# Xjh-UCAS/TAM-TR

Measured on AMD Instinct MI355X. Metric: images/sec fwd+bwd @640x640 bs=16/GPU, higher is better.
Workload: dtype bf16

## Files before the change

### include/tamtr_hip.h

```cpp
#ifndef TAMTR_HIP_H
#define TAMTR_HIP_H

#include <stdint.h>

#ifdef __cplusplus
extern "C" {
#endif

#define TAMTR_F32 0
#define TAMTR_BF16 1

#define TAMTR_OK 0
#define TAMTR_EINVAL (-1)
#define TAMTR_EUNSUP (-2)
#define TAMTR_ELAUNCH (-3)

int tamtr_abi_version(void);

int tamtr_maxsigmoid_gate_fwd(const void* x, const float* gk, const float* bias, const void* v, void* out, float* aw,
                              int32_t* arg, int B, int nh, int hc, int HW, int T, float scale, int dtype, void* stream);

int tamtr_maxsigmoid_gate_bwd(const void* dout, const void* x, const float* gk, const void* v, const float* aw,
                              const int32_t* arg, void* dx, void* dv, float* dlogit, int B, int nh, int hc, int HW, int T,
                              float scale, int dtype, void* stream);
int tamtr_maxsigmoid_gate_cl_fwd(const void* e, long long ld_e, const float* mean_rstd_e, const float* gamma_e, const float* beta_e,
                                 const void* v, const float* mean_rstd_v, const float* gamma_v, const float* beta_v, const float* gk,
                                 const float* bias, void* out, float* aw, int32_t* arg, int B, int nh, int hc, int HW, int T, float scale,
                                 int dtype, void* stream);

int tamtr_conv3x3_tiles(int B, int H, int W);
int tamtr_conv3x3_pack_weight(const void* w, void* wpk, int C1, int C2, int dtype, void* stream);
int tamtr_conv3x3_cl_stats_fwd(const void* x, long long ld_x, const void* wpk, void* y, float* running_mean, float* running_var,
                               float* mean_rstd, float* partials, int B, int H, int W, int C1, int C2, float eps, float momentum,
                               void* stream);
int tamtr_bn_finalize(const float* partials, float* mean_rstd, float* running_mean, float* running_var, int C, int S, float eps,
                      float momentum, void* stream);

int tamtr_msdeform_attn_fwd(const void* value, const int32_t* shapes_host, const float* loc, const float* aw, void* out,
                            int B, int L, int M, int D, int Q, int nl, int P, int dtype, void* stream);

int tamtr_msdeform_attn_bwd(const void* gout, const void* value, const int32_t* shapes_host, const float* loc,
                            const float* aw, float* gvalue, float* gloc, float* gaw, int B, int L, int M, int D, int Q,
                            int nl, int P, int dtype, void* stream);

int tamtr_msdeform_attn_bwd_sorted(const void* gout, const void* value, const int32_t* shapes_host, const float* loc,
                                   const float* aw, void* gvalue, float* gloc, float* gaw, float* colw, int B, int L, int M,
                                   int D, int Q, int nl, int P, long long ldg, int dtype, void* stream);

int tamtr_contrastive_logits_fwd(const void* x, const float* w, const float* logit_scale, const float* bias, float* logits,
                                 float* xinv, float* winv, int B, int Q, int K, int C, int dtype, void* stream);

int tamtr_contrastive_bwd_slabs(int Q);
int tamtr_contrastive_logits_bwd(const float* g, const void* x, const float* w, const float* logit_scale, const float* xinv,
                                 const float* winv, void* dx, float* dwhat, int B, int Q, int K, int C, int dtype,
                                 void* stream);

int tamtr_linear_bf16(const void* X, const void* W, const float* bias, void* Y, int M, int N, int K, void* stream);

int tamtr_selfattn_fwd(const void* q, const void* k, const void* v, const uint32_t* mask_bits, void* o, float* lse, int B,
                       int Q, int nh, int dh, int ldq, int ldk, int ldv, int dtype, void* stream);
int tamtr_selfattn_bwd(const void* go, const void* q, const void* k, const void* v, const void* o, const float* lse,
                       const uint32_t* mask_bits, void* gq, void* gk, void* gv, float* delta_ws, int B, int Q, int nh, int dh,
                       int ldq, int ldk, int ldv, int dtype, void* stream);

int tamtr_selective_scan_chunk(void);
int tamtr_selective_scan_fwd(const float* u, const float* delta, const float* A, const float* Bm, const float* Cm,
                             const float* D, const float* dbias, float* y, float* hstate, int B, int K, int Dk, int N, int L,
                             int xmode, void* stream);
int tamtr_selective_scan_bwd_slabs(int Dk);
int tamtr_selective_scan_row_sums(void);
int tamtr_selective_scan_bwd(const float* gy, const float* u, const float* delta, const float* A, const float* Bm,
                             const float* Cm, const float* D, const float* dbias, const float* hstate, float* gu,
                             float* gdelta, float* grow, float* gB, float* gC, float* ws, int B, int K, int Dk, int N, int L,
                             int xmode, void* stream);

int tamtr_selective_scan_dtproj_fwd(const void* u, const float* dtr, const float* Wdt, const float* A, const float* Bm,
                                    const float* Cm, const float* D, const float* dbias, void* y, float* hstate, int B, int K,
                                    int Dk, int N, int R, int L, int xmode, int planes_bf16, void* stream);
int tamtr_selective_scan_dtproj_bwd(const void* gy, const void* u, const float* dtr, const float* Wdt, const float* A,
                                    const float* Bm, const float* Cm, const float* D, const float* dbias, const float* hstate,
                                    void* gu, void* gdelta_ws, float* gdtr, float* grow, float* gB, float* gC, float* ws, int B,
                                    int K, int Dk, int N, int R, int L, int xmode, int bf16_flags, void* stream);

int tamtr_lsap_assign(const float* cost, const int32_t* group_sizes_host, int bs, int nq, int G, int64_t* batch_idx,
                      int64_t* query_idx, int64_t* gt_idx, void* stream);

int tamtr_cpam_fwd(const void* x, const void* p, void* out, float* s2, int32_t* arg, int B, int C, int H, int W, int dtype,
                   void* stream);

int tamtr_cpam_bwd(const void* gout, const void* x, const void* p, const float* s2, const int32_t* arg, void* dx_direct,
                   void* du_ws, void* dp, int B, int C, int H, int W, int dtype, void* stream);

int tamtr_cpam_cl_fwd(const void* x, void* p, uint8_t* code, void* out, float* s2, int32_t* arg, int B, int C, int H, int W, int dtype, void* stream);
int tamtr_cpam_cl_bwd(const void* gout, const void* x, const void* p, const uint8_t* code, const float* s2, const int32_t* arg, void* dxd_ws,
                      void* du_ws, void* dp_ws, void* dx, int B, int C, int H, int W, int dtype, void* stream);

int tamtr_dwconv_silu_cross_fwd(const void* x, long long x_pixel_stride, const float* weight, const float* bias, void* u2, int B,
                                int D, int H, int W, int dtype, int plane_dtype, void* stream);
int tamtr_dwconv_tiles(int H, int W);
int tamtr_dwconv_silu_cross_bwd(const void* g2, const void* x, long long x_pixel_stride, const float* weight, const float* bias,
                                void* gx, long long gx_pixel_stride, float* ws, int B, int D, int H, int W, int dtype, int plane_dtype,
                                void* stream);

int tamtr_cross_merge_fwd(const void* y4, float* ymT, int B, int D, int H, int W, int plane_dtype, void* stream);
int tamtr_cross_merge_bwd(const float* gymT, void* g2, int B, int D, int H, int W, int plane_dtype, void* stream);

int tamtr_ln_gate_blocks(long long ntok);
int tamtr_ln_gate_fwd(const float* x, const void* xz, long long xz_token_stride, const float* gamma, const float* beta, void* out,
                      float* stats, long long ntok, int D, float eps, int dtype, void* stream);
int tamtr_ln_gate_bwd(const void* gout, const float* x, const void* xz, long long xz_token_stride, const float* gamma,
                      const float* beta, const float* stats, float* gx, void* gxz, float* partials, long long ntok, int D, int dtype,
                      void* stream);

int tamtr_sum_n(const void* const* src, int n, void* out, long long n_elems, int dtype, void* stream);

int tamtr_colsum_blocks(long long M);
int tamtr_colsum_bf16(const void* X, float* partial, long long M, int N, void* stream);
int tamtr_slab_sum_rows(const void* in, float* out, int R, long long C, int dtype, void* stream);
int tamtr_dw_slices(long long M, int N, int K);
int tamtr_dw_bf16(const void* dY, const void* X, float* part, int with_db, long long M, int N, int K, void* stream);
int tamtr_fold_add(const float* g4, const void* m0, const void* m1, float* out, int B, long long n, int dtype, void* stream);

int tamtr_layernorm_fwd(const void* x, const float* gamma, const float* beta, void* out, float* stats, long long ntok, int D,
                        float eps, int dtype, void* stream);
int tamtr_layernorm_bwd(const void* gout, const void* x, const float* gamma, const float* stats, void* gx, float* partials,
                        long long ntok, int D, int dtype, void* stream);

int tamtr_bn_slices(int B, int HW);
int tamtr_bn_act_fwd(const void* x, const float* gamma, const float* beta, float* running_mean, float* running_var, void* y,
                     float* mean_rstd, float* partials, int B, int C, int HW, float eps, float momentum, int act, int dtype, void* stream);
int tamtr_bn_act_bwd(const void* gy, const void* x, const float* gamma, const float* beta, const float* mean_rstd, void* gx,
                     float* ggamma, float* gbeta, float* partials, int B, int C, int HW, int act, int dtype, void* stream);

int tamtr_bncl_blocks(long long N, int C, int dtype);
int tamtr_bncl_act_fwd(const void* x, const float* gamma, const float* beta, float* running_mean, float* running_var, const void* residual,
                       void* y, float* mean_rstd, float* partials, long long N, int C, float eps, float momentum, int act, int dtype,
                       void* stream);
int tamtr_bncl_stats(const void* x, float* running_mean, float* running_var, float* mean_rstd, float* partials, long long N, int C, float eps,
                     float momentum, int dtype, void* stream);
int tamtr_bncl2_act_fwd(const void* x1, const float* gamma1, const float* beta1, float* running_mean1, float* running_var1, const void* x2,
                        const float* gamma2, const float* beta2, float* running_mean2, float* running_var2, void* y, float* mean_rstd,
                        float* partials, long long N, int C, float eps, float momentum, int act, int dtype, void* stream);
int tamtr_bncl2_act_bwd(const void* gy, long long ldgy, const void* x1, const void* x2, const float* gamma1, const float* beta1,
                        const float* gamma2, const float* beta2, const float* mean_rstd, void* gx1, void* gx2, float* ggamma1, float* gbeta1,
                        float* ggamma2, float* gbeta2, float* partials, long long N, int C, int act, int dtype, void* stream);
int tamtr_bncl_act_bwd(const void* gy, long long ldgy, const void* x, const float* gamma, const float* beta, const float* mean_rstd,
                       void* gx, float* ggamma, float* gbeta, float* partials, long long N, int C, int act, int dtype, void* stream);

int tamtr_relayout(const void* src, void* dst, int B, int C, int HW, int ld, int to_nhwc, int dtype, void* stream);
int tamtr_resample2(const void* src, void* dst, int B, int H, int W, int C, int mode, int dtype, void* stream);
int tamtr_copy_rows(const void* src, long long lds, void* dst, long long ldd, long long N, int C, int dtype, void* stream);
int tamtr_cat_rows(const void* const* src, const long long* lds, const int* C, int n, void* dst, long long ldd, long long N, int dtype,
                   void* stream);

int tamtr_maxpool_out(int n, int k, int s, int p);
int tamtr_maxpool_fwd(const void* x, void* y, uint8_t* code, int B, int C, int H, int W, int k, int s, int p, int nhwc, int dtype,
                      void* stream);
int tamtr_maxpool_bwd(const void* gy, const uint8_t* code, const void* addend, void* gx, int B, int C, int H, int W, int k, int s, int p, int nhwc, int dtype,
                      void* stream);

int tamtr_img_augment_u8(const uint8_t* src, const double* inv_affine, const uint8_t* luts, const int32_t* flags, float* out, int B,
                         int SH, int SW, int H, int W, int border, void* stream);

int tamtr_optim_chunk(void);
int tamtr_optim_step(const void* const* p, const void* const* m, const void* const* v, const void* const* e, const void* const* shadow, float* step,
                     const long long* numel,
                     const unsigned char* group, const int* chunk_tensor, const long long* chunk_off, const void* const* grads, int ntensors,
                     int nchunks, float* partial, float* normcoef, const float* lr, const float* wd, int ngroups, float beta1, float beta2, float eps,
                     float max_norm, float ema_decay, int do_ema, void* stream);

int tamtr_xproj_dw_slices(int L);
int tamtr_xproj_fwd(const void* u2, const void* wcat, float* dtr, float* Bs, float* Cs, int B, int D, int L, int R, int plane_dtype, void* stream);
int tamtr_xproj_bwd_dx(const void* gu, const float* gdtr, const float* gB, const float* gC, const void* wT, void* gu2, int B, int D, int L, int R,
                       int plane_dtype, void* stream);
int tamtr_xproj_bwd_dw(const void* u2, const float* gdtr, const float* gB, const float* gC, float* part, int B, int D, int L, int R, int plane_dtype,
                       void* stream);

int tamtr_detr_blocks(int rows_per_layer);
int tamtr_detr_layers_fwd(const float* pb, const float* ps, const float* gt_bboxes, const long long* gt_cls, const long long* li, const long long* bi,
                          const long long* si, const long long* gi, int Lr, int B, int nq, int nc, int n, long long* tgt, float* score, float* pair_l1,
                          float* pair_riou, float* partial, float g_class, float g_bbox, float g_giou, float* out, void* stream);
int tamtr_detr_layers_bwd(const float* pb, const float* ps, const float* gt_bboxes, const long long* li, const long long* bi, const long long* si,
                          const long long* gi, const long long* tgt, const float* score, const float* up, int Lr, int B, int nq, int nc, int n,
                          float g_class, float g_bbox, float g_giou, float* gpb, float* gps, void* stream);
int tamtr_detr_match_cost(const float* ps, const float* pb, const float* gt_bboxes, const long long* gt_cls, long long rows, int nc, int G, float g_class,
// ... 98 lines not shown
```

### tam-tr_amd/_lib.py

```python
import ctypes
import os
from ctypes import c_float, c_int, c_longlong, c_void_p

_HERE = os.path.dirname(os.path.abspath(__file__))
LIB_PATH = os.environ.get('TAMTR_HIP_LIB') or os.path.join(_HERE, 'csrc', 'libtamtr_hip.so')
ABI_VERSION = 36

F32, BF16 = 0, 1
_ERR = {-1: 'TAMTR_EINVAL (bad argument)', -2: 'TAMTR_EUNSUP (shape/dtype outside what the kernels are built for)',
        -3: 'TAMTR_ELAUNCH (HIP launch error)'}


class TamtrHipError(RuntimeError):
    pass


_P, _I, _F, _LL, _D = c_void_p, c_int, c_float, c_longlong, ctypes.c_double
_SIGS = {
    'tamtr_abi_version': [],
    'tamtr_maxsigmoid_gate_fwd': [_P, _P, _P, _P, _P, _P, _P, _I, _I, _I, _I, _I, _F, _I, _P],
    'tamtr_maxsigmoid_gate_bwd': [_P, _P, _P, _P, _P, _P, _P, _P, _P, _I, _I, _I, _I, _I, _F, _I, _P],
    'tamtr_msdeform_attn_fwd': [_P, _P, _P, _P, _P, _I, _I, _I, _I, _I, _I, _I, _I, _P],
    'tamtr_msdeform_attn_bwd': [_P, _P, _P, _P, _P, _P, _P, _P, _I, _I, _I, _I, _I, _I, _I, _I, _P],
    'tamtr_msdeform_attn_bwd_sorted': [_P, _P, _P, _P, _P, _P, _P, _P, _P, _I, _I, _I, _I, _I, _I, _I, _LL, _I, _P],
    'tamtr_contrastive_logits_fwd': [_P, _P, _P, _P, _P, _P, _P, _I, _I, _I, _I, _I, _P],
    'tamtr_contrastive_logits_bwd': [_P, _P, _P, _P, _P, _P, _P, _P, _I, _I, _I, _I, _I, _P],
    'tamtr_contrastive_bwd_slabs': [_I],
    'tamtr_linear_bf16': [_P, _P, _P, _P, _I, _I, _I, _P],
    'tamtr_selfattn_fwd': [_P, _P, _P, _P, _P, _P, _I, _I, _I, _I, _I, _I, _I, _I, _P],
    'tamtr_selfattn_bwd': [_P] * 11 + [_I, _I, _I, _I, _I, _I, _I, _I, _P],
    'tamtr_selective_scan_chunk': [],
    'tamtr_selective_scan_fwd': [_P, _P, _P, _P, _P, _P, _P, _P, _P, _I, _I, _I, _I, _I, _I, _P],
    'tamtr_selective_scan_bwd_slabs': [_I],
    'tamtr_selective_scan_row_sums': [],
    'tamtr_selective_scan_bwd': [_P] * 15 + [_I, _I, _I, _I, _I, _I, _P],
    'tamtr_selective_scan_dtproj_fwd': [_P] * 10 + [_I] * 8 + [_P],
    'tamtr_selective_scan_dtproj_bwd': [_P] * 17 + [_I] * 8 + [_P],
    'tamtr_lsap_assign': [_P, _P, _I, _I, _I, _P, _P, _P, _P],
    'tamtr_img_augment_u8': [_P, _P, _P, _P, _P, _I, _I, _I, _I, _I, _I, _P],
    'tamtr_cpam_fwd': [_P, _P, _P, _P, _P, _I, _I, _I, _I, _I, _P],
    'tamtr_cpam_cl_fwd': [_P, _P, _P, _P, _P, _P, _I, _I, _I, _I, _I, _P],
    'tamtr_cpam_bwd': [_P] * 8 + [_I, _I, _I, _I, _I, _P],
    'tamtr_cpam_cl_bwd': [_P] * 10 + [_I, _I, _I, _I, _I, _P],
    'tamtr_dwconv_silu_cross_fwd': [_P, _LL, _P, _P, _P, _I, _I, _I, _I, _I, _I, _P],
    'tamtr_dwconv_tiles': [_I, _I],
    'tamtr_cross_merge_fwd': [_P, _P, _I, _I, _I, _I, _I, _P],
    'tamtr_cross_merge_bwd': [_P, _P, _I, _I, _I, _I, _I, _P],
    'tamtr_ln_gate_blocks': [_LL],
    'tamtr_bn_slices': [_I, _I],
    'tamtr_maxpool_out': [_I, _I, _I, _I],
    'tamtr_maxpool_fwd': [_P, _P, _P, _I, _I, _I, _I, _I, _I, _I, _I, _I, _P],
    'tamtr_maxpool_bwd': [_P, _P, _P, _P, _I, _I, _I, _I, _I, _I, _I, _I, _I, _P],
    'tamtr_sum_n': [_P, _I, _P, _LL, _I, _P],
    'tamtr_colsum_blocks': [_LL],
    'tamtr_colsum_bf16': [_P, _P, _LL, _I, _P],
    'tamtr_fold_add': [_P, _P, _P, _P, _I, _LL, _I, _P],
    'tamtr_slab_sum_rows': [_P, _P, _I, _LL, _I, _P],
    'tamtr_dw_slices': [_LL, _I, _I],
    'tamtr_dw_bf16': [_P, _P, _P, _I, _LL, _I, _I, _P],
    'tamtr_graph_capture_census': [_P, _P, _I],
    'tamtr_box_refine_fwd': [_P, _P, _P, _LL, _P],
    'tamtr_box_refine_bwd': [_P, _P, _P, _P, _P, _LL, _P],
    'tamtr_bncl_act_seg_fwd': [_P, _P, _P, _P, _P, _P, _LL, _LL, _P, _P, _LL, _I, _F, _F, _I, _I, _P],
    'tamtr_bncl_act_seg_bwd': [_P, _LL, _LL, _P, _P, _P, _P, _P, _P, _P, _P, _LL, _I, _I, _I, _P],
    'tamtr_detr_blocks': [_I],
    'tamtr_detr_layers_fwd': [_P] * 8 + [_I] * 5 + [_P] * 5 + [_F, _F, _F, _P, _P],
    'tamtr_detr_layers_bwd': [_P] * 10 + [_I] * 5 + [_F, _F, _F, _P, _P, _P],
    'tamtr_detr_match_cost': [_P, _P, _P, _P, _LL, _I, _I, _F, _F, _F, _F, _F, _P, _P],
    'tamtr_xproj_dw_slices': [_I],
    'tamtr_xproj_fwd': [_P, _P, _P, _P, _P, _I, _I, _I, _I, _I, _P],
    'tamtr_xproj_bwd_dx': [_P, _P, _P, _P, _P, _P, _I, _I, _I, _I, _I, _P],
    'tamtr_xproj_bwd_dw': [_P, _P, _P, _P, _P, _I, _I, _I, _I, _I, _P],
    'tamtr_optim_chunk': [],
    'tamtr_optim_step': [_P] * 11 + [_I, _I, _P, _P, _P, _P, _I, _F, _F, _F, _F, _F, _I, _P],
    'tamtr_resample2': [_P, _P, _I, _I, _I, _I, _I, _I, _P],
    'tamtr_cat_rows': [_P, _P, _P, _I, _P, _LL, _LL, _I, _P],
    'tamtr_copy_rows': [_P, _LL, _P, _LL, _LL, _I, _I, _P],
    'tamtr_relayout': [_P, _P, _I, _I, _I, _I, _I, _I, _P],
    'tamtr_bncl_blocks': [_LL, _I, _I],
    'tamtr_bncl_act_fwd': [_P, _P, _P, _P, _P, _P, _P, _P, _P, _LL, _I, _F, _F, _I, _I, _P],
    'tamtr_bncl_stats': [_P, _P, _P, _P, _P, _LL, _I, _F, _F, _I, _P],
    'tamtr_bn_finalize': [_P, _P, _P, _P, _I, _I, _F, _F, _P],
    'tamtr_conv3x3_tiles': [_I, _I, _I],
    'tamtr_conv3x3_pack_weight': [_P, _P, _I, _I, _I, _P],
    'tamtr_conv3x3_cl_stats_fwd': [_P, _LL, _P, _P, _P, _P, _P, _P, _I, _I, _I, _I, _I, _F, _F, _P],
    'tamtr_maxsigmoid_gate_cl_fwd': [_P, _LL, _P, _P, _P, _P, _P, _P, _P, _P, _P, _P, _P, _P, _I, _I, _I, _I, _I, _F, _I, _P],
    'tamtr_bncl2_act_fwd': [_P, _P, _P, _P, _P, _P, _P, _P, _P, _P, _P, _P, _P, _LL, _I, _F, _F, _I, _I, _P],
    'tamtr_bncl2_act_bwd': [_P, _LL, _P, _P, _P, _P, _P, _P, _P, _P, _P, _P, _P, _P, _P, _P, _LL, _I, _I, _I, _P],
    'tamtr_bncl_act_bwd': [_P, _LL, _P, _P, _P, _P, _P, _P, _P, _P, _LL, _I, _I, _I, _P],
    'tamtr_bn_act_fwd': [_P, _P, _P, _P, _P, _P, _P, _P, _I, _I, _I, _F, _F, _I, _I, _P],
    'tamtr_bn_act_bwd': [_P, _P, _P, _P, _P, _P, _P, _P, _P, _I, _I, _I, _I, _I, _P],
    'tamtr_layernorm_fwd': [_P, _P, _P, _P, _P, _LL, _I, _F, _I, _P],
    'tamtr_layernorm_bwd': [_P, _P, _P, _P, _P, _P, _LL, _I, _I, _P],
    'tamtr_ln_gate_fwd': [_P, _P, _LL, _P, _P, _P, _P, _LL, _I, _F, _I, _P],
    'tamtr_ln_gate_bwd': [_P, _P, _P, _LL, _P, _P, _P, _P, _P, _P, _LL, _I, _I, _P],
    'tamtr_dwconv_silu_cross_bwd': [_P, _P, _LL, _P, _P, _P, _LL, _P, _I, _I, _I, _I, _I, _I, _P],
    'tamtr_detect_postprocess': [_P, _I, _I, _I, _I, _P, _F, _F, _I, _F, _P, _I, _P, _P, _P, _P],
    'tamtr_val_postprocess_match': [_P, _I, _I, _I, _I, _F, _F, _F, _I, _F, _P, _P, _P, _I, _P, _P, _P, _P, _P],
    'tamtr_val_confusion': [_P, _P, _I, _I, _I, _P, _P, _P, _I, _P, _F, _F, _P, _P],
    'tamtr_val_ap_tile': [],
    'tamtr_val_ap_curves': [_P, _P, _P, _I, _I, _P, _I] + [_P] * 10 + [_P],
    'tamtr_text_embed': [_P, _P, _P, _P, _LL, _I, _I, _I, _P],
    'tamtr_linear_f32': [_P, _P, _P, _P, _P, _I, _I, _I, _I, _P],
    'tamtr_text_pool_project': [_P, _P, _P, _P, _P, _P, _I, _I, _I, _I, _F, _I, _P],
    'tamtr_bytetrack_update': [_P, _P, _I, _I, _P, _P, _P, _P, _P, _I, _F, _F, _F, _D, _I, _P, _P, _P, _I, _P],
    'tamtr_bytetrack_workspace_bytes': [_I, _I],
    'tamtr_botsort_update': [_P, _P, _P, _I, _I, _P, _P, _P, _P, _P, _I, _F, _F, _F, _D, _I, _P, _P, _P, _I, _P],
    'tamtr_botsort_reid_update': [_P, _P, _P, _P, _I, _I, _P, _P, _P, _P, _P, _P, _I, _I, _F, _F, _F, _D, _I, _F, _D, _P, _P, _P, _I, _P],
    'tamtr_botsort_reid_workspace_bytes': [_I, _I],
    'tamtr_reid_rows': [_P, _I, _P, _P, _I, _I, _I, _I, _P, _P],
    'tamtr_gmc_workspace_bytes': [_I, _I, _I],
    'tamtr_gmc_workspace_offset': [_I, _I, _I, _I],
    'tamtr_gmc_state_bytes': [_I, _I],
    'tamtr_gmc_estimate': [_P, _P, _P, _I, _I, _I, _P, _P, _P, _P, _P, _P, _I, _I, _P],
    'tamtr_val_coco_match': [_P, _P, _I, _I, _I, _P, _P, _P, _I, _P, _P, _I, _P, _P, _P, _P, _I, _P],
    'tamtr_val_coco_workspace_bytes': [_I, _I, _I],
    'tamtr_val_coco_accumulate': [_P, _P, _P, _I, _I, _P, _P, _I, _P, _P, _P, _P, _P],
    'tamtr_mot_update': [_P, _P, _P, _P, _I, _I, _I, _I, _D, _P, _P, _P, _P, _P, _I, _I, _P, _I, _P],
    'tamtr_mot_end_sequence': [_I, _P, _P, _P, _P, _I, _I, _I, _P, _I, _P],
    'tamtr_mot_workspace_bytes': [_I, _I, _I, _I, _I],
    'tamtr_hota_update': [_P, _P, _P, _P, _I, _I, _I, _I, _D, _D, _P, _P, _P, _I, _P],
    'tamtr_hota_end_sequence': [_P, _D, _I, _I, _I, _I, _P, _P, _P, _I, _P],
    'tamtr_hota_workspace_bytes': [_I, _I, _I],
    'tamtr_trackmap_update': [_P, _P, _P, _P, _I, _I, _I, _I, _D, _P, _P, _P, _I, _P],
    'tamtr_trackmap_end_sequence': [_P, _I, _D, _I, _P, _P, _P, _I, _P],
    'tamtr_trackmap_workspace_bytes': [_I, _I, _I, _I, _I, _I],
}
EXPORTS = tuple(_SIGS)
# ... 49 lines not shown
```

### tam-tr_amd/csrc/dwconv.hip

```cpp
#include "common.h"

namespace {

constexpr int TS = 16;
constexpr int DW_THREADS = TS * TS;
#ifndef DW_CB_BWD
#define DW_CB_BWD 16
#endif
constexpr int CB_FWD = 32, CB_BWD = DW_CB_BWD;

__device__ __forceinline__ float silu_f(float v) { return v / (1.f + __expf(-v)); }

template <typename T>
struct Vec16;
template <>
struct Vec16<float> {
  static constexpr int N = 4;
  static __device__ __forceinline__ void ld(const float* p, float (&o)[4]) {
    const float4 v = *reinterpret_cast<const float4*>(p);
    o[0] = v.x; o[1] = v.y; o[2] = v.z; o[3] = v.w;
  }
  static __device__ __forceinline__ void st(float* p, const float (&v)[4]) { *reinterpret_cast<float4*>(p) = make_float4(v[0], v[1], v[2], v[3]); }
};
template <>
// ... 183 lines not shown
      }
#pragma unroll
      for (int k = 0; k < GB; ++k) {
        const int it = threadIdx.x + (k0 + k) * DW_THREADS;
        if (it < CB * GS * GS) {
          const int c = it / (GS * GS), r = it - c * (GS * GS), px = r / GS, py = r - px * GS;
          s_g[c][py][px] += v[k];
        }
      }
    }
  }
  }
#endif
  __syncthreads();
#ifndef DW_ABL_NOSILU
  {
    constexpr int TPC = DW_THREADS / CB;
    static_assert(DW_THREADS % CB == 0 && TPC <= WAVE && (TPC & (TPC - 1)) == 0, "a power-of-two lane group per channel");
    const int c = threadIdx.x / TPC, sub = threadIdx.x % TPC;
    float wk[9], dwk[10];
#pragma unroll
    for (int k9 = 0; k9 < 9; ++k9) { wk[k9] = s_w[c][k9]; dwk[k9] = 0.f; }
    dwk[9] = 0.f;
    const float bc = s_w[c][9];
    for (int r = sub; r < GS * GS; r += TPC) {
      const int px = r / GS, py = r - px * GS;
      const int h = h0 + py - 1, w = w0 + px - 1;
      float g = 0.f;
      if (h >= 0 && h < H && w >= 0 && w < W) {
        g = s_g[c][py][px];
        float xin[9], acc = bc;
#pragma unroll
        for (int ky = 0; ky < 3; ++ky)
#pragma unroll
          for (int kx = 0; kx < 3; ++kx) { xin[ky * 3 + kx] = s_x[c][py + ky][px + kx]; acc = fmaf(wk[ky * 3 + kx], xin[ky * 3 + kx], acc); }
        const float sg = 1.f / (1.f + __expf(-acc));
        g *= sg * (1.f + acc * (1.f - sg));
        if (py >= 1 && py <= TS && px >= 1 && px <= TS) {
#pragma unroll
          for (int k9 = 0; k9 < 9; ++k9) dwk[k9] = fmaf(g, xin[k9], dwk[k9]);
          dwk[9] += g;
        }
      }
      s_g[c][py][px] = g;
    }
#pragma unroll
    for (int k9 = 0; k9 < 10; ++k9) dwk[k9] = group_sum<TPC>(dwk[k9]);
    if (sub == 0) {
      float* o = ws + (((size_t)b * tiles + blockIdx.x) * D + d0 + c) * 10;
#pragma unroll
      for (int k9 = 0; k9 < 10; ++k9) o[k9] = dwk[k9];
    }
  }
#endif
  __syncthreads();
  const int ty = threadIdx.x / TS, tx = threadIdx.x % TS;
  float dxv[CB];
#pragma unroll
  for (int c = 0; c < CB; ++c) {
    float acc = 0.f;
#pragma unroll
    for (int ky = 0; ky < 3; ++ky)
#pragma unroll
      for (int kx = 0; kx < 3; ++kx) acc = fmaf(s_w[c][ky * 3 + kx], s_g[c][ty + 2 - ky][tx + 2 - kx], acc);
    dxv[c] = acc;
  }
  __syncthreads();
#pragma unroll
  for (int c = 0; c < CB; ++c) s_x[c][ty][tx] = dxv[c];
  __syncthreads();
  constexpr int VN = Vec16<T>::N, GROUPS = CB / VN;
  for (int it = threadIdx.x; it < TS * TS * GROUPS; it += DW_THREADS) {
    const int pix = it / GROUPS, gq = it - pix * GROUPS, py = pix / TS, px = pix - py * TS;
    const int h = h0 + py, w = w0 + px;
    if (h < H && w < W) {
      float v[VN];
#pragma unroll
      for (int j = 0; j < VN; ++j) v[j] = s_x[gq * VN + j][py][px];
      Vec16<T>::st(gx + ((size_t)(b * H + h) * W + w) * gxs + d0 + gq * VN, v);
    }
  }
}

}

static int dwconv_check(const void* a, const void* b, const void* c, int B, int D, int H, int W, long long xs, int dtype) {
  if (!a || !b || !c || B <= 0 || D <= 0 || H <= 0 || W <= 0 || xs < D) return TAMTR_EINVAL;
  if (dtype != TAMTR_F32 && dtype != TAMTR_BF16) return TAMTR_EINVAL;
  const int vn = dtype == TAMTR_F32 ? 4 : 8;
  if (D % CB_FWD || xs % vn || B > 65535 || D / CB_BWD > 65535) return TAMTR_EUNSUP;
  return TAMTR_OK;
}

extern "C" int tamtr_dwconv_silu_cross_fwd(const void* x, long long x_pixel_stride, const float* weight, const float* bias, void* u2,
                                           int B, int D, int H, int W, int dtype, int plane_dtype, void* stream) {
  const int rc = dwconv_check(x, weight, u2, B, D, H, W, x_pixel_stride, dtype);
  if (rc) return rc;
  if (plane_dtype != TAMTR_F32 && !(plane_dtype == TAMTR_BF16 && dtype == TAMTR_BF16)) return TAMTR_EINVAL;
  const int tiles_w = (W + TS - 1) / TS, tiles_h = (H + TS - 1) / TS;
  const dim3 grid(tiles_w * tiles_h, D / CB_FWD, B);
  hipStream_t s = (hipStream_t)stream;
  if (dtype == TAMTR_F32)
    hipLaunchKernelGGL((dwconv_cross_fwd_kernel<float, float>), grid, dim3(DW_THREADS), 0, s, (const float*)x, (size_t)x_pixel_stride, weight, bias,
                       (float*)u2, D, H, W, tiles_w);
  else if (plane_dtype == TAMTR_F32)
    hipLaunchKernelGGL((dwconv_cross_fwd_kernel<bf16_t, float>), grid, dim3(DW_THREADS), 0, s, (const bf16_t*)x, (size_t)x_pixel_stride, weight,
                       bias, (float*)u2, D, H, W, tiles_w);
  else
    hipLaunchKernelGGL((dwconv_cross_fwd_kernel<bf16_t, bf16_t>), grid, dim3(DW_THREADS), 0, s, (const bf16_t*)x, (size_t)x_pixel_stride, weight,
                       bias, (bf16_t*)u2, D, H, W, tiles_w);
  return tamtr_launch_status();
}

extern "C" int tamtr_dwconv_tiles(int H, int W) { return ((W + TS - 1) / TS) * ((H + TS - 1) / TS); }

extern "C" int tamtr_dwconv_silu_cross_bwd(const void* g2, const void* x, long long x_pixel_stride, const float* weight, const float* bias,
                                           void* gx, long long gx_pixel_stride, float* ws, int B, int D, int H, int W, int dtype,
                                           int plane_dtype, void* stream) {
  const int rc = dwconv_check(x, weight, g2, B, D, H, W, x_pixel_stride, dtype);
  if (rc) return rc;
  if (!gx || !ws || gx_pixel_stride < D || gx_pixel_stride % (dtype == TAMTR_F32 ? 4 : 8)) return TAMTR_EINVAL;
  if (plane_dtype != TAMTR_F32 && !(plane_dtype == TAMTR_BF16 && dtype == TAMTR_BF16)) return TAMTR_EINVAL;
  if ((uintptr_t)g2 % 16) return TAMTR_EUNSUP;
  const int tiles_w = (W + TS - 1) / TS, tiles_h = (H + TS - 1) / TS;
  const dim3 grid(tiles_w * tiles_h, D / CB_BWD, B);
  hipStream_t s = (hipStream_t)stream;
  if (dtype == TAMTR_F32)
    hipLaunchKernelGGL((dwconv_cross_bwd_kernel<float, float>), grid, dim3(DW_THREADS), 0, s, (const float*)g2, (const float*)x, (size_t)x_pixel_stride,
                       weight, bias, (float*)gx, (size_t)gx_pixel_stride, ws, D, H, W, tiles_w, tiles_w * tiles_h);
  else if (plane_dtype == TAMTR_F32)
    hipLaunchKernelGGL((dwconv_cross_bwd_kernel<bf16_t, float>), grid, dim3(DW_THREADS), 0, s, (const float*)g2, (const bf16_t*)x,
                       (size_t)x_pixel_stride, weight, bias, (bf16_t*)gx, (size_t)gx_pixel_stride, ws, D, H, W, tiles_w, tiles_w * tiles_h);
  else
    hipLaunchKernelGGL((dwconv_cross_bwd_kernel<bf16_t, bf16_t>), grid, dim3(DW_THREADS), 0, s, (const bf16_t*)g2, (const bf16_t*)x,
                       (size_t)x_pixel_stride, weight, bias, (bf16_t*)gx, (size_t)gx_pixel_stride, ws, D, H, W, tiles_w, tiles_w * tiles_h);
  return tamtr_launch_status();
}
```

### tam-tr_amd/ops.py

```python
import ctypes
import math

import torch

from . import _lib
from ._lib import call, dtype_code, ptr, require_gpu, stream_ptr
import os as _os

_PROJ_CONV_LIB = _os.environ.get('TAMTR_PROJ_CONV') == 'miopen'

_I, _F = ctypes.c_int, ctypes.c_float


def _c(t):
    return t if t.is_contiguous() else t.contiguous()


def _is_cl(t):
    return t.dim() == 4 and not t.is_contiguous() and t.is_contiguous(memory_format=torch.channels_last)


def is_cl(t):
    return _is_cl(t)

# ... 1120 lines not shown
        _, gA, gD, gbias = _split_row_sums(grow, 0)
        return (_fold_directions(gu) if ctx.xmode else gu), gdelta, gA, gB, gC, gD, gbias, None


def selective_scan(u, delta, A, Bm, Cm, D, delta_bias):
    return _SelectiveScan.apply(u, delta, A, Bm, Cm, D, delta_bias, 0)


def selective_scan_cross_delta(u2, delta, A, Bm, Cm, D, delta_bias):
    return _SelectiveScan.apply(u2, delta, A, Bm, Cm, D, delta_bias, 1)


def _plane_dtype(pc):
    return torch.bfloat16 if pc else torch.float32


def _scan_dtproj_fwd(u, dtr, Wdt, A, Bm, Cm, D, dbias, xmode, pc):
    Bn, K, R, L = dtr.shape
    KD, N = A.shape
    y = torch.empty(Bn, KD, L, device=u.device, dtype=_plane_dtype(pc))
    hstate = _scan_hstate(Bn, KD, L, N, u.device)
    call('tamtr_selective_scan_dtproj_fwd', ptr(u), ptr(dtr), ptr(Wdt), ptr(A), ptr(Bm), ptr(Cm), ptr(D), ptr(dbias), ptr(y),
         ptr(hstate), Bn, K, KD // K, N, R, L, xmode, pc, stream_ptr())
    return y, hstate


def _scan_dtproj_bwd(gy, u, dtr, Wdt, A, Bm, Cm, D, dbias, hstate, xmode, ws16, pc):
    Bn, K, R, L = dtr.shape
    KD, N = A.shape
    gu = torch.empty(Bn, KD, L, device=u.device, dtype=_plane_dtype(pc))
    gdelta = torch.empty(Bn, KD, L, device=u.device, dtype=_plane_dtype(ws16))
    gdtr = torch.empty_like(dtr)
    gB, gC = torch.empty_like(Bm), torch.empty_like(Cm)
    grow = _scan_row_sums(Bn, KD, u.device)
    ws = _scan_bwd_slabs(Bm, KD // K)
    call('tamtr_selective_scan_dtproj_bwd', ptr(gy), ptr(u), ptr(dtr), ptr(Wdt), ptr(A), ptr(Bm), ptr(Cm), ptr(D), ptr(dbias),
         ptr(hstate), ptr(gu), ptr(gdelta), ptr(gdtr), ptr(grow), ptr(gB), ptr(gC), ptr(ws), Bn, K,
         KD // K, N, R, L, xmode, int(bool(ws16)) | (2 * pc), stream_ptr())
    return (gu, gdtr, gB, gC) + _split_row_sums(grow, R)


class _SelectiveScanDtProj(torch.autograd.Function):

    @staticmethod
    def forward(ctx, u, dtr, Wdt, A, Bm, Cm, D, dbias, xmode):
        require_gpu(u, dtr, Wdt, A, Bm, Cm, D, dbias)
        u, dtr, Wdt, A, Bm, Cm, D, dbias = (_c(t.float()) for t in (u, dtr, Wdt, A, Bm, Cm, D, dbias))
        y, hstate = _scan_dtproj_fwd(u, dtr, Wdt, A, Bm, Cm, D, dbias, int(xmode), 0)
        ctx.save_for_backward(u, dtr, Wdt, A, Bm, Cm, D, dbias, hstate)
        ctx.xmode = int(xmode)
        return y

    @staticmethod
    def backward(ctx, gy):
        gy = _c(gy.float())
        gu, gdtr, gB, gC, gW, gA, gD, gbias = _scan_dtproj_bwd(gy, *ctx.saved_tensors, ctx.xmode, False, 0)
        return (_fold_directions(gu) if ctx.xmode else gu), gdtr, gW, gA, gB, gC, gD, gbias, None


class _CrossScanInput(torch.autograd.Function):

    @staticmethod
    def forward(ctx, xc):
        B, D, H, W = xc.shape
        a = torch.nn.functional.silu(xc)
        u2 = torch.empty(B, 2, D, H * W, device=xc.device, dtype=torch.float32)
        u2[:, 0].view(B, D, H, W).copy_(a)
        u2[:, 1].view(B, D, W, H).copy_(a.transpose(2, 3))
        ctx.save_for_backward(xc)
        return u2

    @staticmethod
    def backward(ctx, g2):
        (xc,) = ctx.saved_tensors
        B, D, H, W = xc.shape
        ga = g2[:, 0].view(B, D, H, W) + g2[:, 1].view(B, D, W, H).transpose(2, 3)
        return torch.ops.aten.silu_backward(ga.to(xc.dtype), xc)


def cross_scan_input(xc):
    return _CrossScanInput.apply(xc)


def _dwconv_silu_cross_fwd(xz, weight, bias, D, pc):
    B, H, W, C2 = xz.shape
    w = _c(weight.float().reshape(D, 9))
    bvec = _c(bias.float()) if bias is not None else None
    u2 = torch.empty(B, 2, D, H * W, device=xz.device, dtype=_plane_dtype(pc))
    call('tamtr_dwconv_silu_cross_fwd', ptr(xz), C2, ptr(w), ptr(bvec), ptr(u2), B, D, H, W, dtype_code(xz), pc, stream_ptr())
    return u2, w, bvec


def _dwconv_silu_cross_bwd(g2, xz, w, bvec, gxz, pc, w_shape, w_dt, b_dt):
    B, H, W, C2 = xz.shape
    D = w.shape[0]
    tiles = _lib.lib().tamtr_dwconv_tiles(H, W)
    ws = torch.empty(B, tiles, D, 10, device=xz.device, dtype=torch.float32)
    call('tamtr_dwconv_silu_cross_bwd', ptr(g2), ptr(xz), C2, ptr(w), ptr(bvec if b_dt is not None else None), ptr(gxz), C2,
         ptr(ws), B, D, H, W, dtype_code(xz), pc, stream_ptr())
    gwb = slab_sum(ws.view(-1, D, 10))
    return gwb[:, :9].reshape(w_shape).to(w_dt), (gwb[:, 9].to(b_dt) if b_dt is not None else None)


class _DWConvSiluCross(torch.autograd.Function):

    @staticmethod
    def forward(ctx, xz, weight, bias, D):
        require_gpu(xz, weight)
        xz = _c(xz)
        u2, w, bvec = _dwconv_silu_cross_fwd(xz, weight, bias, D, 0)
        ctx.save_for_backward(xz, w, bvec if bvec is not None else w.new_empty(0))
        ctx.cfg = (weight.shape, weight.dtype, None if bias is None else bias.dtype)
        return u2

    @staticmethod
    def backward(ctx, g2):
        xz, w, bvec = ctx.saved_tensors
        gxz = torch.zeros_like(xz)
        gw, gb = _dwconv_silu_cross_bwd(_c(g2.float()), xz, w, bvec, gxz, 0, *ctx.cfg)
        return gxz, gw, gb, None


def dwconv_silu_cross(xz, weight, bias, D):
    return _DWConvSiluCross.apply(xz, weight, bias, D)


def _split_len(L, min_len=1024, max_split=16):
    S = 1
    while S < max_split and L % (2 * S) == 0 and L // (2 * S) >= min_len:
        S *= 2
    return S


def _xproj_torch_fwd(wx, u2, cdt, R, N):
    C = R + 2 * N
    ub = u2.to(cdt)
    wa, wb = torch.cat([wx[0], wx[2]], 0).to(cdt), torch.cat([wx[1], wx[3]], 0).to(cdt)
    with torch.autocast('cuda', enabled=False):
        xa, xb = torch.matmul(wa, ub[:, 0]), torch.matmul(wb, ub[:, 1])
    parts = tuple(torch.stack([xa[:, lo:lo + n], xb[:, lo:lo + n], xa[:, C + lo:C + lo + n], xb[:, C + lo:C + lo + n]], 1).float()
                  for lo, n in ((0, R), (R, N), (R + N, N)))
    return parts, ub, wa, wb


def _xproj_torch_bwd(gdtr, gBs, gCs, ub, wa, wb, R, N, gu2=None):
    Bn, _, D, L = ub.shape
    C = R + 2 * N
    S = _split_len(L)
    gws, ms = [], []
    with torch.autocast('cuda', enabled=False):
        for i, w in ((0, wa), (1, wb)):
            gx = torch.cat([gdtr[:, i], gBs[:, i], gCs[:, i], gdtr[:, i + 2], gBs[:, i + 2], gCs[:, i + 2]], 1).to(ub.dtype)
            m = torch.matmul(w.t(), gx)
            if gu2 is None:
                ms.append(m)
            else:
                gu2[:, i].copy_(m)
            ga = gx.view(Bn, 2 * C, S, L // S).transpose(1, 2).reshape(Bn * S, 2 * C, L // S)
            ua = ub[:, i].reshape(Bn, D, S, L // S).transpose(1, 2).reshape(Bn * S, D, L // S)
            gws.append(slab_sum(torch.bmm(ga, ua.transpose(1, 2))))
    return ms, gws


def _xproj_unstack_wgrad(gws, C, dt):
    return torch.stack([gws[0][:C], gws[1][:C], gws[0][C:], gws[1][C:]], 0).to(dt)


class _XProjCross(torch.autograd.Function):

    @staticmethod
    def forward(ctx, wx, u2, R, N):
        cdt = torch.get_autocast_dtype('cuda') if torch.is_autocast_enabled('cuda') else torch.float32
# ... 1285 lines not shown
```

Baseline: 215.4.

## Add blocked bf16 depthwise conv+SiLU cross-scan forward kernels with 32x32 tiles

Adds specialized bf16 forward kernels for the depthwise 3x3 conv + SiLU + cross-scan layout. Each thread computes 8 contiguous outputs from a register window and writes 16-byte vector stores. Both the row-major plane and the transposed plane are emitted, with the transpose done through LDS. A 32x32-tile variant stages bf16 in dynamic LDS, transposes per wavefront using only wave-level fences, and is used when tile padding is small. The aim is fewer redundant halo loads and better-coalesced stores. The cost is large LDS use per block, which may reduce occupancy, and an env flag can fall back to the old kernel.

```diff
diff --git a/include/tamtr_hip.h b/include/tamtr_hip.h
--- a/include/tamtr_hip.h
+++ b/include/tamtr_hip.h
@@ -101,6 +101,8 @@
 int tamtr_dwconv_silu_cross_bwd(const void* g2, const void* x, long long x_pixel_stride, const float* weight, const float* bias,
                                 void* gx, long long gx_pixel_stride, float* ws, int B, int D, int H, int W, int dtype, int plane_dtype,
                                 void* stream);
+#define TAMTR_DW_UNBLOCKED 0x100
+int tamtr_dwconv_blocked_ok(int D, int H, int W, long long x_pixel_stride, int dtype, int plane_dtype);
 
 int tamtr_cross_merge_fwd(const void* y4, float* ymT, int B, int D, int H, int W, int plane_dtype, void* stream);
 int tamtr_cross_merge_bwd(const float* gymT, void* g2, int B, int D, int H, int W, int plane_dtype, void* stream);
diff --git a/tam-tr_amd/_lib.py b/tam-tr_amd/_lib.py
--- a/tam-tr_amd/_lib.py
+++ b/tam-tr_amd/_lib.py
@@ -44,6 +44,7 @@
     'tamtr_cpam_cl_bwd': [_P] * 10 + [_I, _I, _I, _I, _I, _P],
     'tamtr_dwconv_silu_cross_fwd': [_P, _LL, _P, _P, _P, _I, _I, _I, _I, _I, _I, _P],
     'tamtr_dwconv_tiles': [_I, _I],
+    'tamtr_dwconv_blocked_ok': [_I, _I, _I, _LL, _I, _I],
     'tamtr_cross_merge_fwd': [_P, _P, _I, _I, _I, _I, _I, _P],
     'tamtr_cross_merge_bwd': [_P, _P, _I, _I, _I, _I, _I, _P],
     'tamtr_ln_gate_blocks': [_LL],
diff --git a/tam-tr_amd/csrc/dwconv.hip b/tam-tr_amd/csrc/dwconv.hip
--- a/tam-tr_amd/csrc/dwconv.hip
+++ b/tam-tr_amd/csrc/dwconv.hip
@@ -289,6 +289,182 @@
   }
 }
 
+constexpr int BLK_P = 20;
+
+struct Taps {
+  float w[9], bias;
+};
+__device__ __forceinline__ Taps taps_ld(const float* sw) {
+  const float4 a = *reinterpret_cast<const float4*>(sw), b = *reinterpret_cast<const float4*>(sw + 4);
+  const float4 c = *reinterpret_cast<const float4*>(sw + 8);
+  return Taps{{a.x, a.y, a.z, a.w, b.x, b.y, b.z, b.w, c.x}, c.y};
+}
+__device__ __forceinline__ void taps_stage(const float* __restrict__ wgt, const float* __restrict__ bias, int d0, int CB, float (*s_w)[12]) {
+  for (int i = threadIdx.x; i < CB * 12; i += DW_THREADS) {
+    const int c = i / 12, k = i - c * 12;
+    s_w[c][k] = k < 9 ? wgt[(size_t)(d0 + c) * 9 + k] : (k == 9 && bias ? bias[d0 + c] : 0.f);
+  }
+}
+__device__ __forceinline__ void row10_ld(const float* p, float (&o)[10]) {
+  const float4 a = *reinterpret_cast<const float4*>(p), b = *reinterpret_cast<const float4*>(p + 4);
+  const float2 c = *reinterpret_cast<const float2*>(p + 8);
+  o[0] = a.x; o[1] = a.y; o[2] = a.z; o[3] = a.w; o[4] = b.x; o[5] = b.y; o[6] = b.z; o[7] = b.w; o[8] = c.x; o[9] = c.y;
+}
+
+__global__ __launch_bounds__(DW_THREADS) void dwconv_cross_fwd_blocked_kernel(const bf16_t* __restrict__ x, size_t xs,
+                                                                               const float* __restrict__ wgt, const float* __restrict__ bias,
+                                                                               bf16_t* __restrict__ u2, int D, int H, int W, int tiles_w) {
+  constexpr int CB = CB_FWD, SIDE = TS + 2, P = BLK_P, N_IT = CB * 32 / DW_THREADS;
+  __shared__ __attribute__((aligned(16))) float s_in[CB][SIDE][P];
+  __shared__ __attribute__((aligned(16))) float s_w[CB][12];
+  const int th = blockIdx.x / tiles_w, tw = blockIdx.x - th * tiles_w;
+  const int d0 = blockIdx.y * CB, b = blockIdx.z, h0 = th * TS, w0 = tw * TS;
+  const size_t L = (size_t)H * W;
+  taps_stage(wgt, bias, d0, CB, s_w);
+  stage_tile<bf16_t, CB, 1, P>(x, xs, b, d0, h0, w0, H, W, s_in);
+  __syncthreads();
+  const int cw = threadIdx.x / 32, r = (threadIdx.x % 32) / 2, q = (threadIdx.x % 2) * 8;
+  float res[N_IT][8];
+#pragma unroll
+  for (int it = 0; it < N_IT; ++it) {
+    const int c = it * (DW_THREADS / 32) + cw;
+    const Taps t = taps_ld(s_w[c]);
+    float win[3][10];
+#pragma unroll
+    for (int ky = 0; ky < 3; ++ky) row10_ld(&s_in[c][r + ky][q], win[ky]);
+#pragma unroll
+    for (int j = 0; j < 8; ++j) {
+      float acc = t.bias;
+#pragma unroll
+      for (int ky = 0; ky < 3; ++ky)
+#pragma unroll
+        for (int kx = 0; kx < 3; ++kx) acc = fmaf(t.w[ky * 3 + kx], win[ky][j + kx], acc);
+      res[it][j] = silu_f(acc);
+    }
+    if (h0 + r < H && w0 + q < W) Vec16<bf16_t>::st(u2 + ((size_t)(b * 2 + 0) * D + d0 + c) * L + (size_t)(h0 + r) * W + w0 + q, res[it]);
+  }
+  __syncthreads();
+  float (*s_t)[TS][P] = reinterpret_cast<float (*)[TS][P]>(&s_in[0][0][0]);
+#pragma unroll
+  for (int it = 0; it < N_IT; ++it) {
+    const int c = it * (DW_THREADS / 32) + cw;
+#pragma unroll
+    for (int j = 0; j < 8; ++j) s_t[c][q + j][r] = res[it][j];
+  }
+  __syncthreads();
+#pragma unroll
+  for (int it = 0; it < N_IT; ++it) {
+    const int c = it * (DW_THREADS / 32) + cw;
+    const float4 a = *reinterpret_cast<const float4*>(&s_t[c][r][q]), e = *reinterpret_cast<const float4*>(&s_t[c][r][q + 4]);
+    const float v[8] = {a.x, a.y, a.z, a.w, e.x, e.y, e.z, e.w};
+    if (w0 + r < W && h0 + q < H) Vec16<bf16_t>::st(u2 + ((size_t)(b * 2 + 1) * D + d0 + c) * L + (size_t)(w0 + r) * H + h0 + q, v);
+  }
+}
+
+constexpr int T32 = 32, F32_SIDE = T32 + 2, F32_ROW = 36, F32_CH = 2456, F32_CB = 32;
+static_assert(F32_SIDE * F32_ROW * 2 <= F32_CH && T32 * F32_ROW * 2 <= F32_CH && F32_CH % 8 == 0, "a channel's tile and its transposed result fit its stride");
+constexpr size_t F32_LDS = (size_t)F32_CB * F32_CH;
+
+__device__ __forceinline__ float bf_lo(uint32_t v) { return __uint_as_float(v << 16); }
+__device__ __forceinline__ float bf_hi(uint32_t v) { return __uint_as_float(v & 0xffff0000u); }
+__device__ __forceinline__ void wave_lds_fence() {
+  __builtin_amdgcn_fence(__ATOMIC_ACQ_REL, "wavefront");
+  __builtin_amdgcn_wave_barrier();
+}
+
+__global__ __launch_bounds__(DW_THREADS) void dwconv_cross_fwd_blocked32_kernel(const bf16_t* __restrict__ x, size_t xs,
+                                                                                 const float* __restrict__ wgt, const float* __restrict__ bias,
+                                                                                 bf16_t* __restrict__ u2, int D, int H, int W, int tiles_w) {
+  extern __shared__ __attribute__((aligned(16))) unsigned char s_tile[];
+  const int th = blockIdx.x / tiles_w, tw = blockIdx.x - th * tiles_w;
+  const int d0 = blockIdx.y * F32_CB, b = blockIdx.z, h0 = th * T32, w0 = tw * T32;
+  const size_t L = (size_t)H * W;
+  {
+    constexpr int GROUPS = F32_CB / 8, TOTAL = F32_SIDE * F32_SIDE * GROUPS, N_IT = (TOTAL + DW_THREADS - 1) / DW_THREADS;
+    uint4 v[N_IT];
+#pragma unroll
+    for (int k = 0; k < N_IT; ++k) {
+      const int it = min((int)threadIdx.x + k * DW_THREADS, TOTAL - 1);
+      const int pix = it / GROUPS, gq = it - pix * GROUPS, py = pix / F32_SIDE, px = pix - py * F32_SIDE;
+      const int h = min(max(h0 + py - 1, 0), H - 1), w = min(max(w0 + px - 1, 0), W - 1);
+      v[k] = *reinterpret_cast<const uint4*>(x + ((size_t)(b * H + h) * W + w) * xs + d0 + gq * 8);
+    }
+#pragma unroll
+    for (int k = 0; k < N_IT; ++k) {
+      const int it = threadIdx.x + k * DW_THREADS;
+      if (it < TOTAL) {
+        const int pix = it / GROUPS, gq = it - pix * GROUPS, py = pix / F32_SIDE, px = pix - py * F32_SIDE;
+        const int h = h0 + py - 1, w = w0 + px - 1;
+        const bool keep = h >= 0 && h < H && w >= 0 && w < W;
+        const uint32_t wd[4] = {v[k].x, v[k].y, v[k].z, v[k].w};
+        unsigned char* p = s_tile + (size_t)(gq * 8) * F32_CH + (py * F32_ROW + px) * 2;
+#pragma unroll
+        for (int j = 0; j < 8; ++j) {
+          const uint32_t e = (j & 1) ? wd[j / 2] >> 16 : wd[j / 2] & 0xffffu;
+          *reinterpret_cast<bf16_t*>(p + j * F32_CH) = keep ? (bf16_t)e : (bf16_t)0;
+        }
+      }
+    }
+  }
+  __syncthreads();
+  const int lane = threadIdx.x % WAVE, wv = __builtin_amdgcn_readfirstlane(threadIdx.x / WAVE);
+  const int rr = lane / 4, q = (lane % 4) * 8;
+#pragma unroll 1
+  for (int i = 0; i < F32_CB / (DW_THREADS / WAVE); ++i) {
+    const int c = wv * (F32_CB / (DW_THREADS / WAVE)) + i;
+    unsigned char* ch = s_tile + (size_t)c * F32_CH;
+    float wk[9];
+#pragma unroll
+    for (int k9 = 0; k9 < 9; ++k9) wk[k9] = wgt[(size_t)(d0 + c) * 9 + k9];
+    const float bc = bias ? bias[d0 + c] : 0.f;
+    uint32_t pk[2][4];
+#pragma unroll
+    for (int sub = 0; sub < 2; ++sub) {
+      const int r = sub * 16 + rr;
+      float win[3][10];
+#pragma unroll
+      for (int ky = 0; ky < 3; ++ky) {
+        const unsigned char* p = ch + ((r + ky) * F32_ROW + q) * 2;
+        const uint2 a = *reinterpret_cast<const uint2*>(p), e = *reinterpret_cast<const uint2*>(p + 8);
+        const uint32_t f = *reinterpret_cast<const uint32_t*>(p + 16);
+        win[ky][0] = bf_lo(a.x); win[ky][1] = bf_hi(a.x); win[ky][2] = bf_lo(a.y); win[ky][3] = bf_hi(a.y);
+        win[ky][4] = bf_lo(e.x); win[ky][5] = bf_hi(e.x); win[ky][6] = bf_lo(e.y); win[ky][7] = bf_hi(e.y);
+        win[ky][8] = bf_lo(f); win[ky][9] = bf_hi(f);
+      }
+      float res[8];
+#pragma unroll
+      for (int j = 0; j < 8; ++j) {
+        float acc = bc;
+#pragma unroll
+        for (int ky = 0; ky < 3; ++ky)
+#pragma unroll
+          for (int kx = 0; kx < 3; ++kx) acc = fmaf(wk[ky * 3 + kx], win[ky][j + kx], acc);
+        res[j] = silu_f(acc);
+      }
+#pragma unroll
+      for (int j = 0; j < 4; ++j) pk[sub][j] = (uint32_t)f2bf(res[2 * j]) | ((uint32_t)f2bf(res[2 * j + 1]) << 16);
+      if (h0 + r < H && w0 + q < W)
+        *reinterpret_cast<uint4*>(u2 + ((size_t)(b * 2 + 0) * D + d0 + c) * L + (size_t)(h0 + r) * W + w0 + q) =
+            make_uint4(pk[sub][0], pk[sub][1], pk[sub][2], pk[sub][3]);
+    }
+    wave_lds_fence();
+#pragma unroll
+    for (int sub = 0; sub < 2; ++sub)
+#pragma unroll
+      for (int j = 0; j < 8; ++j)
+        *reinterpret_cast<bf16_t*>(ch + ((q + j) * F32_ROW + sub * 16 + rr) * 2) = (bf16_t)((j & 1) ? pk[sub][j / 2] >> 16 : pk[sub][j / 2] & 0xffffu);
+    wave_lds_fence();
+#pragma unroll
+    for (int k = 0; k < 2; ++k) {
+      const int item = k * WAVE + lane, xc = item / 4, ys = (item % 4) * 8;
+      const unsigned char* p = ch + (xc * F32_ROW + ys) * 2;
+      const uint2 a = *reinterpret_cast<const uint2*>(p), e = *reinterpret_cast<const uint2*>(p + 8);
+      if (w0 + xc < W && h0 + ys < H)
+        *reinterpret_cast<uint4*>(u2 + ((size_t)(b * 2 + 1) * D + d0 + c) * L + (size_t)(w0 + xc) * H + h0 + ys) = make_uint4(a.x, a.y, e.x, e.y);
+    }
+  }
+}
+
 }
 
 static int dwconv_check(const void* a, const void* b, const void* c, int B, int D, int H, int W, long long xs, int dtype) {
@@ -299,15 +475,33 @@
   return TAMTR_OK;
 }
 
+extern "C" int tamtr_dwconv_blocked_ok(int D, int H, int W, long long x_pixel_stride, int dtype, int plane_dtype) {
+  return dtype == TAMTR_BF16 && plane_dtype == TAMTR_BF16 && D > 0 && D % CB_FWD == 0 && x_pixel_stride >= D && x_pixel_stride % 8 == 0 &&
+         H > 0 && W > 0 && H % 8 == 0 && W % 8 == 0;
+}
+
 extern "C" int tamtr_dwconv_silu_cross_fwd(const void* x, long long x_pixel_stride, const float* weight, const float* bias, void* u2,
                                            int B, int D, int H, int W, int dtype, int plane_dtype, void* stream) {
   const int rc = dwconv_check(x, weight, u2, B, D, H, W, x_pixel_stride, dtype);
   if (rc) return rc;
+  const bool parent = plane_dtype & TAMTR_DW_UNBLOCKED;
+  plane_dtype &= ~TAMTR_DW_UNBLOCKED;
   if (plane_dtype != TAMTR_F32 && !(plane_dtype == TAMTR_BF16 && dtype == TAMTR_BF16)) return TAMTR_EINVAL;
   const int tiles_w = (W + TS - 1) / TS, tiles_h = (H + TS - 1) / TS;
   const dim3 grid(tiles_w * tiles_h, D / CB_FWD, B);
   hipStream_t s = (hipStream_t)stream;
-  if (dtype == TAMTR_F32)
+  const bool blocked = !parent && tamtr_dwconv_blocked_ok(D, H, W, x_pixel_stride, dtype, plane_dtype) && (uintptr_t)u2 % 16 == 0;
+  const long long pad32 = (long long)((H + T32 - 1) / T32) * ((W + T32 - 1) / T32) * T32 * T32;
+  if (blocked && 2 * pad32 <= 3LL * H * W) {
+    const int t32w = (W + T32 - 1) / T32, t32h = (H + T32 - 1) / T32;
+    if (hipFuncSetAttribute((const void*)dwconv_cross_fwd_blocked32_kernel, hipFuncAttributeMaxDynamicSharedMemorySize, (int)F32_LDS) != hipSuccess)
+      return TAMTR_ELAUNCH;
+    hipLaunchKernelGGL(dwconv_cross_fwd_blocked32_kernel, dim3(t32w * t32h, D / F32_CB, B), dim3(DW_THREADS), F32_LDS, s, (const bf16_t*)x,
+                       (size_t)x_pixel_stride, weight, bias, (bf16_t*)u2, D, H, W, t32w);
+  } else if (blocked)
+    hipLaunchKernelGGL(dwconv_cross_fwd_blocked_kernel, grid, dim3(DW_THREADS), 0, s, (const bf16_t*)x, (size_t)x_pixel_stride, weight, bias,
+                       (bf16_t*)u2, D, H, W, tiles_w);
+  else if (dtype == TAMTR_F32)
     hipLaunchKernelGGL((dwconv_cross_fwd_kernel<float, float>), grid, dim3(DW_THREADS), 0, s, (const float*)x, (size_t)x_pixel_stride, weight, bias,
                        (float*)u2, D, H, W, tiles_w);
   else if (plane_dtype == TAMTR_F32)
diff --git a/tam-tr_amd/ops.py b/tam-tr_amd/ops.py
--- a/tam-tr_amd/ops.py
+++ b/tam-tr_amd/ops.py
@@ -1226,12 +1226,25 @@
     return _CrossScanInput.apply(xc)
 
 
+_DWCONV_BLOCKED = _os.environ.get('TAMTR_DWCONV_BLOCKED') != '0'
+_DW_UNBLOCKED = 0x100
+
+
+def dwconv_blocked(xz, D, pc):
+    _, H, W, C2 = xz.shape
+    return _DWCONV_BLOCKED and bool(_lib.lib().tamtr_dwconv_blocked_ok(D, H, W, C2, dtype_code(xz), pc))
+
+
+def _dw_plane_code(pc):
+    return pc if _DWCONV_BLOCKED else pc | _DW_UNBLOCKED
+
+
 def _dwconv_silu_cross_fwd(xz, weight, bias, D, pc):
     B, H, W, C2 = xz.shape
     w = _c(weight.float().reshape(D, 9))
     bvec = _c(bias.float()) if bias is not None else None
     u2 = torch.empty(B, 2, D, H * W, device=xz.device, dtype=_plane_dtype(pc))
-    call('tamtr_dwconv_silu_cross_fwd', ptr(xz), C2, ptr(w), ptr(bvec), ptr(u2), B, D, H, W, dtype_code(xz), pc, stream_ptr())
+    call('tamtr_dwconv_silu_cross_fwd', ptr(xz), C2, ptr(w), ptr(bvec), ptr(u2), B, D, H, W, dtype_code(xz), _dw_plane_code(pc), stream_ptr())
     return u2, w, bvec
 
 
```

Result: no change. 215.8, median of 5 (+0.2%).
